# Ryukhaan/speech-to-video-mpp

Hardware: AMD Instinct MI355X
Metric: synthesized 256×256 frames/sec/GPU (LNet+ENet path); 1/2/4/8-GPU scaling (higher is better)
Workload: dtype f32; 1 GPU; ENet(+LNet) forward, B=16 synthetic 256x256 crops + [1,80,16] mel windows -> 384x384 (models/ENet.py:82-139); crop=256, global_batch=16, batch_per_gpu=16, parallelism=frame-shard x1 (no data-path collective), graph=True, lanes=1, world_size_seen=1

## Files before the change

### include/s2v.h

```cpp
#ifndef S2V_H_
#define S2V_H_

#include <stddef.h>
#include <stdint.h>

#ifdef __cplusplus
extern "C" {
#endif

typedef void *s2v_stream_t;

enum {
    S2V_OK = 0,
    S2V_E_INVALID = -1,
    S2V_E_LAUNCH = -2,
    S2V_E_WORKSPACE = -3
};

enum {
    S2V_ACT_NONE = 0,
    S2V_ACT_RELU = 1,
    S2V_ACT_LRELU = 2,
    S2V_ACT_SIGMOID = 3,
    S2V_ACT_TANH = 4,
// ... 85 lines not shown
                      float eps, float post, float *d, int d_ns, s2v_stream_t stream);

int s2v_modconv_demod_rows(const float *s, int batch, int s_ns, const int *rows, int nrows,
                           const float *wsq, float eps, float post, float *d, int d_ns,
                           s2v_stream_t stream);

int s2v_resize(const float *x, int n, int c, int ih, int iw, long long xsn, long long xsc, long long xsy,
               long long xsx, float *y, int oh, int ow, long long ysn, long long ysc, long long ysy,
               long long ysx, float scale_h, float scale_w, int mode, s2v_stream_t stream);

int s2v_torgb_up2(const float *x, int n, int h, int w, int c, int xcs, const float *wt, int kpad, const float *s,
                  int s_ns, const float *bias, const float *skip, int skcs, float *y, int ycs, s2v_stream_t stream);

typedef struct s2v_torgb_win {
    int fh, fw;
    int oy, ox;
    int sh, sw;
    int sy, sx;
    int nchw, cy, cx;
} s2v_torgb_win;
int s2v_torgb_up2_win(const float *x, int n, int h, int w, int c, int xcs, const float *wt, int kpad, const float *s,
                      int s_ns, const float *bias, const float *skip, int skcs, float *y, int ycs,
                      const s2v_torgb_win *win, s2v_stream_t stream);

int s2v_row_pack(const float *x, int n, int h, int w, int c, int xcs, int kw, int pw, float *y, int ycs,
                 s2v_stream_t stream);

int s2v_pad_reflect(const float *x, int n, int h, int w, int c, int xcs, int pt, int pb, int pl, int pr,
                    float *y, int ycs, s2v_stream_t stream);

int s2v_row_layernorm(const float *x, int rows, int dim, int xld, const float *weight, const float *bias,
                      float eps, float *y, int yld, s2v_stream_t stream);

int s2v_attention(const float *q, const float *k, const float *v, int batch, int heads, int tokens,
                  int dim_head, int ld_q, int ld_k, int ld_v, long long bs_q, long long bs_k, long long bs_v,
                  float scale, float *o, int ld_o, long long bs_o, s2v_stream_t stream);

int s2v_flow_warp(const float *flow, int n, int fh, int fw, int flow_cs, const float *src, int c, int h,
                  int w, long long ssn, long long ssc, long long ssy, long long ssx, float *y, int ycs,
                  s2v_stream_t stream);
int s2v_flow_warp_cat(const float *flow, int n, int fh, int fw, int flow_cs, const float *src, int c, int h,
                      int w, long long ssn, long long ssc, long long ssy, long long ssx, float *y, int ycs,
                      s2v_stream_t stream);

int s2v_melspectrogram(const float *wav, long long n_samples, const float *tables, int pad_reflect,
                       float *out, long long frames, s2v_stream_t stream);
// ... 186 lines not shown
```

### speech-to-video-mpp_amd/_lib.py

```python
from __future__ import annotations

import ctypes
import os
import threading

LIB_PATH = os.path.join(os.path.dirname(os.path.abspath(__file__)), "libs2v.so")

ACT_NONE, ACT_RELU, ACT_LRELU, ACT_SIGMOID, ACT_TANH, ACT_GELU_TANH = range(6)
IN_DIRECT, IN_NEAREST_UP2, IN_TRANSPOSED = range(3)
PAD_ZERO, PAD_REFLECT = range(2)
PREC_F32, PREC_BF16X3, PREC_F16X3, PREC_F16 = range(4)

_c_int, _c_float, _c_ll, _c_size, _vp = ctypes.c_int, ctypes.c_float, ctypes.c_longlong, ctypes.c_size_t, ctypes.c_void_p


class ConvParams(ctypes.Structure):
    _fields_ = [
        ("x", _vp), ("n", _c_int), ("h", _c_int), ("w", _c_int), ("cin", _c_int), ("xcs", _c_int),
        ("in_mode", _c_int), ("pad_mode", _c_int), ("pre_act", _c_int), ("pre_alpha", _c_float),
        ("in_scale", _vp), ("in_scale_ns", _c_int),
        ("kh", _c_int), ("kw", _c_int), ("sh", _c_int), ("sw", _c_int), ("ph", _c_int), ("pw", _c_int),
        ("dh", _c_int), ("dw", _c_int),
        ("wt", _vp), ("kpad", _c_int), ("npad", _c_int), ("cout", _c_int), ("b_kn", _c_int), ("ldb", _c_int),
        ("y", _vp), ("oh", _c_int), ("ow", _c_int), ("ycs", _c_int),
# ... 24 lines not shown
    "s2v_conv2d": (_c_int, [ctypes.POINTER(ConvParams), _vp]),
    "s2v_conv2d_ws_bytes": (_c_size, [ctypes.POINTER(ConvParams)]),
    "s2v_conv2d_plan": (_c_int, [ctypes.POINTER(ConvParams), ctypes.POINTER(_c_int)]),
    "s2v_conv2d_group": (_c_int, [ctypes.POINTER(ConvParams), _c_int, _vp]),
    "s2v_conv2d_group_ws_bytes": (_c_size, [ctypes.POINTER(ConvParams), _c_int]),
    "s2v_conv2d_group_plan": (_c_int, [ctypes.POINTER(ConvParams), _c_int, ctypes.POINTER(_c_int)]),
    "s2v_tune": (_c_int, [_c_int, _c_ll, ctypes.POINTER(_c_ll)]),
    "s2v_layernorm2d": (_c_int, [_vp, _c_int, _c_int, _c_int, _c_int, _c_int, _vp, _vp, _c_float, _c_int, _c_float,
                                 _c_int, _vp, _c_int, _vp, _c_int, _vp, _c_size, _vp]),
    "s2v_layernorm2d_ws_bytes": (_c_size, [_c_int, _c_int, _c_int, _c_int]),
    "s2v_instnorm_adain": (_c_int, [_vp, _c_int, _c_int, _c_int, _c_int, _c_int, _vp, _vp, _c_int, _c_float, _c_int,
                                    _c_float, _vp, _c_int, _vp, _c_int, _vp, _c_size, _vp]),
    "s2v_instnorm_adain_pad": (_c_int, [_vp, _c_int, _c_int, _c_int, _c_int, _c_int, _vp, _vp, _c_int, _c_float,
                                        _c_int, _c_float, _vp, _c_int, _vp, _c_int, _vp, _c_int, _vp, _c_size, _vp]),
    "s2v_instnorm_ws_bytes": (_c_size, [_c_int, _c_int, _c_int, _c_int]),
    "s2v_adain_params": (_c_int, [_vp, _c_int, _c_int, _c_int, _vp, _vp, _vp, _c_int, _vp, _c_int, _vp]),
    "s2v_modconv_demod": (_c_int, [_vp, _c_int, _c_int, _c_int, _vp, _c_int, _c_float, _c_float, _vp, _c_int, _vp]),
    "s2v_modconv_demod_rows": (_c_int, [_vp, _c_int, _c_int, _vp, _c_int, _vp, _c_float, _c_float, _vp, _c_int,
                                        _vp]),
    "s2v_torgb_up2": (_c_int, [_vp, _c_int, _c_int, _c_int, _c_int, _c_int, _vp, _c_int, _vp, _c_int, _vp, _vp,
                               _c_int, _vp, _c_int, _vp]),
    "s2v_torgb_up2_win": (_c_int, [_vp, _c_int, _c_int, _c_int, _c_int, _c_int, _vp, _c_int, _vp, _c_int, _vp, _vp,
                                   _c_int, _vp, _c_int, _vp, _vp]),
    "s2v_resize": (_c_int, [_vp, _c_int, _c_int, _c_int, _c_int, _c_ll, _c_ll, _c_ll, _c_ll, _vp, _c_int, _c_int,
                            _c_ll, _c_ll, _c_ll, _c_ll, _c_float, _c_float, _c_int, _vp]),
    "s2v_row_pack": (_c_int, [_vp, _c_int, _c_int, _c_int, _c_int, _c_int, _c_int, _c_int, _vp, _c_int, _vp]),
    "s2v_pad_reflect": (_c_int, [_vp, _c_int, _c_int, _c_int, _c_int, _c_int, _c_int, _c_int, _c_int, _c_int, _vp,
                                 _c_int, _vp]),
    "s2v_row_layernorm": (_c_int, [_vp, _c_int, _c_int, _c_int, _vp, _vp, _c_float, _vp, _c_int, _vp]),
    "s2v_attention": (_c_int, [_vp, _vp, _vp, _c_int, _c_int, _c_int, _c_int, _c_int, _c_int, _c_int, _c_ll, _c_ll,
                               _c_ll, _c_float, _vp, _c_int, _c_ll, _vp]),
    "s2v_flow_warp": (_c_int, [_vp, _c_int, _c_int, _c_int, _c_int, _vp, _c_int, _c_int, _c_int, _c_ll, _c_ll,
                               _c_ll, _c_ll, _vp, _c_int, _vp]),
    "s2v_flow_warp_cat": (_c_int, [_vp, _c_int, _c_int, _c_int, _c_int, _vp, _c_int, _c_int, _c_int, _c_ll, _c_ll,
                                   _c_ll, _c_ll, _vp, _c_int, _vp]),
    "s2v_melspectrogram": (_c_int, [_vp, _c_ll, _vp, _c_int, _vp, _c_ll, _vp]),
    "s2v_mel_chunks": (_c_int, [_vp, _c_ll, _vp, _c_int, _c_int, _vp, _vp]),
    "s2v_fused_bias_act": (_c_int, [_vp, _vp, _vp, _vp, _c_ll, _c_int, _c_ll, _c_int, _c_int, _c_float, _c_float,
                                    _vp]),
    "s2v_upfirdn2d": (_c_int, [_vp, _c_int, _c_int, _c_int, _c_int, _vp, _c_int, _c_int, _c_int, _c_int, _c_int,
                               _c_int, _c_int, _c_int, _c_int, _c_int, _vp, _c_int, _c_int, _vp]),
    "s2v_fused_bias_act_dt": (_c_int, [_c_int, _vp, _vp, _vp, _vp, _c_ll, _c_int, _c_ll, _c_int, _c_int,
                                       ctypes.c_double, ctypes.c_double, _vp]),
    "s2v_upfirdn2d_dt": (_c_int, [_c_int, _vp, _c_int, _c_int, _c_int, _c_int, _vp, _c_int, _c_int, _c_int, _c_int,
                                  _c_int, _c_int, _c_int, _c_int, _c_int, _c_int, _vp, _c_int, _c_int, _vp]),
    "s2v_fir2d": (_c_int, [_vp, _c_int, _c_int, _c_int, _c_int, _c_int, _vp, _c_int, _c_int, _c_int, _c_int, _c_int,
# ... 132 lines not shown
```

### speech-to-video-mpp_amd/csrc/torch_launch.cpp

```cpp
#include <ATen/ATen.h>
#include <ATen/hip/HIPContext.h>
#include <c10/core/DeviceGuard.h>
#include <torch/library.h>

#include <vector>

#include "../../include/s2v.h"

namespace {

using at::Tensor;
using OptT = c10::optional<Tensor>;

void *stream() { return (void *)at::hip::getCurrentHIPStream().stream(); }

void check(int rc, const char *what) { TORCH_CHECK(rc == 0, what, " failed (", rc, "): ", s2v_last_error()); }

bool has(const OptT &t) { return t && t->defined(); }

void same_dev(const Tensor &t, const at::Device &dev, const char *what) {
    TORCH_CHECK(t.is_cuda(), what, ": expected a HIP device tensor (the s2v ops have no CPU kernel)");
    TORCH_CHECK(t.device() == dev, what, ": on ", t.device(), ", the op's inputs are on ", dev);
}

// ... 674 lines not shown
    } else {
        for (int64_t v : window) TORCH_CHECK(v >= 0 && v < (1 << 30), "torgb window: bad value ", v);
        win.fh = (int)window[0]; win.fw = (int)window[1]; win.oy = (int)window[2]; win.ox = (int)window[3];
        win.sy = (int)window[4]; win.sx = (int)window[5];
    }
    float *yp = nullptr;
    int ycs = 0;
    if (crop.empty()) {
        const NV yv = nhwc(y, dev, "torgb y");
        TORCH_CHECK(yv.n == xv.n && yv.h == xv.h && yv.w == xv.w && yv.c == 4, "torgb: y [N, H, W, 4] view expected");
        yp = yv.p; ycs = yv.cs;
    } else {
        f32(y, dev, "torgb y");
        TORCH_CHECK(crop[0] >= 0 && crop[1] >= 0 && 2 * crop[0] < xv.h && 2 * crop[1] < xv.w, "torgb crop: bad (cy, cx)");
        win.nchw = 1; win.cy = (int)crop[0]; win.cx = (int)crop[1];
        TORCH_CHECK(y.dim() == 4 && y.is_contiguous() && y.size(0) == xv.n && y.size(1) == 3 &&
                        y.size(2) == xv.h - 2 * win.cy && y.size(3) == xv.w - 2 * win.cx,
                    "torgb: contiguous NCHW y [N, 3, H - 2 cy, W - 2 cx] expected, got ", y.sizes());
        yp = y.data_ptr<float>();
    }
    check(s2v_torgb_up2_win(xv.p, xv.n, xv.h, xv.w, xv.c, xv.cs, wt.data_ptr<float>(), (int)wt.size(1),
                            s.data_ptr<float>(), s_ns, bp, kv.p, kv.cs, yp, ycs, &win, stream()),
          "s2v_torgb_up2");
}

void flow_warp_(const Tensor &flow, const Tensor &src, const Tensor &y) {
    const c10::DeviceGuard guard(flow.device());
    const at::Device dev = flow.device();
    const NV fv = nhwc(flow, dev, "flow_warp flow"), yv = nhwc(y, dev, "flow_warp y");
    f32(src, dev, "flow_warp src");
    TORCH_CHECK(src.dim() == 4 && src.size(0) == fv.n && fv.c >= 2, "flow_warp: src [N, C, H, W], flow >= 2 channels");
    TORCH_CHECK(yv.n == fv.n && yv.h == src.size(2) && yv.w == src.size(3) && yv.c == src.size(1), "flow_warp: y shape");
    check(s2v_flow_warp(fv.p, fv.n, fv.h, fv.w, fv.cs, src.data_ptr<float>(), (int)src.size(1), (int)src.size(2),
                        (int)src.size(3), src.stride(0), src.stride(1), src.stride(2), src.stride(3), yv.p, yv.cs,
                        stream()),
          "s2v_flow_warp");
}

void flow_warp_cat_(const Tensor &flow, const Tensor &src, const Tensor &y) {
    const c10::DeviceGuard guard(flow.device());
    const at::Device dev = flow.device();
    const NV fv = nhwc(flow, dev, "flow_warp_cat flow"), yv = nhwc(y, dev, "flow_warp_cat y");
    f32(src, dev, "flow_warp_cat src");
    TORCH_CHECK(src.dim() == 4 && src.size(0) == fv.n && fv.c >= 2, "flow_warp_cat: src [N, C, H, W], flow >= 2 channels");
    TORCH_CHECK(yv.n == fv.n && yv.h == src.size(2) && yv.w == src.size(3) && yv.c == 2 * src.size(1),
                "flow_warp_cat: y [N, H, W, 2C]");
// ... 293 lines not shown
    m.def("group_abort_() -> ()", &group_abort_);
    m.def("group_end_(Tensor? ws, bool dry) -> int[]", &group_end_);
    m.def("gemm_kn_(Tensor a, Tensor b, Tensor(a!) out, int batch, int a_bs, int b_bs, int out_bs, Tensor? res, "
          "int res_bs, int act, float alpha, int prec, Tensor? ws, int force_tile, int force_splits, bool dry) -> int[]");
    m.def("split_weights_(Tensor w, Tensor(a!) out, int prec, float scale) -> ()");
    m.def("split_act_(Tensor x, Tensor(a!) out, int prec) -> ()");
    m.def("layernorm2d_(Tensor x, Tensor weight, Tensor bias, float eps, int act, float alpha, bool pool, "
          "Tensor? res, Tensor(a!) y, Tensor? ws) -> int");
    m.def("instnorm_(Tensor x, Tensor? gamma, Tensor? beta, float eps, int act, float alpha, Tensor? res, "
          "Tensor(a!) y, Tensor(b!)? pad_out, Tensor? ws) -> int");
    m.def("adain_params_(Tensor hid, int nhidden, Tensor w2t, Tensor bias, Tensor seg, Tensor(a!) out) -> ()");
    m.def("modconv_demod_(Tensor s, Tensor wsq, Tensor(a!) d, float eps, float post) -> ()");
    m.def("modconv_demod_rows_(Tensor s, Tensor rows, Tensor wsq, Tensor(a!) d, float eps, float post, "
          "int s_reach) -> ()");
    m.def("row_layernorm_(Tensor x, Tensor weight, Tensor bias, float eps, Tensor(a!) y) -> ()");
    m.def("attention_(Tensor q, Tensor k, Tensor v, Tensor(a!) out, int batch, int heads, int tokens, int dim_head, "
          "float scale) -> ()");
    m.def("resize_(Tensor x, int x_off, int[4] x_size, int[4] x_stride, Tensor(a!) y, int y_off, int[4] y_size, "
          "int[4] y_stride, float scale_h, float scale_w, int mode) -> ()");
    m.def("pad_reflect_(Tensor x, Tensor(a!) y, int[4] pads) -> ()");
    m.def("row_pack_(Tensor x, Tensor(a!) y, int kw, int pw) -> ()");
    m.def("torgb_up2_(Tensor x, Tensor wt, Tensor s, Tensor? bias, Tensor skip, Tensor(a!) y, int[] window, "
          "int[] crop) -> ()");
    m.def("flow_warp_(Tensor flow, Tensor src, Tensor(a!) y) -> ()");
    m.def("flow_warp_cat_(Tensor flow, Tensor src, Tensor(a!) y) -> ()");
    m.def("fill_value_(Tensor(a!) y, float value) -> ()");
    m.def("gaussian_noise_(Tensor(a!) y, int seed, int offset, Tensor? ctr, int shift) -> ()");
    m.def("counter_add_(Tensor(a!) ctr, int inc) -> ()");
    m.def("rfft2_(Tensor x, Tensor tables, Tensor(a!) spec) -> ()");
    m.def("irfft2_(Tensor spec, Tensor tables, Tensor? res, Tensor(a!) y) -> ()");
    m.def("ffc_spec_fwd_(Tensor x_g, Tensor w1, float wt_scale, float x_scale, Tensor? scale, Tensor? shift, "
          "Tensor tables, Tensor(a!) t1, Tensor(b!) spec, Tensor? flag, int prec) -> ()");
    m.def("ffc_spec_inv_(Tensor spec, Tensor wfu, float wt_scale, float x_scale, Tensor? scale, Tensor? shift, "
          "Tensor tables, Tensor t1, Tensor(a!) u, Tensor? flag, int prec) -> ()");
    m.def("ffc_norm_(Tensor(c!) y, Tensor u, Tensor w2, float wt_scale, float x_scale, Tensor? gamma, Tensor? beta, "
          "float eps, int act, float alpha, Tensor? res, Tensor(a!) out, Tensor(b!)? pad_out, Tensor? flag, int prec) -> ()");
    m.def("eltwise_(Tensor x, Tensor? mul, Tensor? add, Tensor? bias, float a, int act, float alpha, float post, "
          "Tensor(a!) y) -> ()");
    m.def("fir2d_(Tensor x, Tensor kernel, Tensor(a!) y, int up, int down, int pad_y0, int pad_x0, float gain, "
          "Tensor? bias, int act, float alpha, float post) -> ()");
    m.def("lipsync_inputs_(Tensor src, Tensor? fake, Tensor(a!) ref_u8, Tensor(b!) face6, Tensor(c!) gt) -> ()");
    m.def("to_u8_(Tensor x, Tensor(a!) y, float lo, float hi, float scale, float offset) -> ()");
    m.def("mel_chunks_(Tensor mel, Tensor starts, int step, Tensor(a!) out) -> ()");
    m.def("melspectrogram_(Tensor wav, Tensor tables, bool pad_reflect, Tensor(a!) out) -> ()");
}

TORCH_LIBRARY_IMPL(s2v, CUDA, m) {
    m.impl("conv2d_", &conv2d_);
    m.impl("modulated_conv2d_", &modulated_conv2d_);
    m.impl("modulate_weights_", &modulate_weights_);
    m.impl("gemm_kn_", &gemm_kn_);
    m.impl("split_weights_", &split_weights_);
    m.impl("amax_", &amax_);
    m.impl("split_act_", &split_act_);
    m.impl("layernorm2d_", &layernorm2d_);
    m.impl("instnorm_", &instnorm_);
    m.impl("adain_params_", &adain_params_);
    m.impl("modconv_demod_", &modconv_demod_);
    m.impl("modconv_demod_rows_", &modconv_demod_rows_);
    m.impl("row_layernorm_", &row_layernorm_);
    m.impl("attention_", &attention_);
    m.impl("resize_", &resize_);
    m.impl("pad_reflect_", &pad_reflect_);
    m.impl("row_pack_", &row_pack_);
    m.impl("torgb_up2_", &torgb_up2_);
    m.impl("flow_warp_", &flow_warp_);
    m.impl("flow_warp_cat_", &flow_warp_cat_);
    m.impl("fill_value_", &fill_value_);
    m.impl("gaussian_noise_", &gaussian_noise_);
    m.impl("counter_add_", &counter_add_);
    m.impl("rfft2_", &rfft2_);
    m.impl("irfft2_", &irfft2_);
    m.impl("ffc_spec_fwd_", &ffc_spec_fwd_);
    m.impl("ffc_spec_inv_", &ffc_spec_inv_);
    m.impl("ffc_norm_", &ffc_norm_);
    m.impl("eltwise_", &eltwise_);
    m.impl("fir2d_", &fir2d_);
    m.impl("lipsync_inputs_", &lipsync_inputs_);
    m.impl("to_u8_", &to_u8_);
    m.impl("mel_chunks_", &mel_chunks_);
    m.impl("melspectrogram_", &melspectrogram_);
}
```

### speech-to-video-mpp_amd/csrc/torgb.hip

```cpp
#include "common.hpp"

namespace s2v {

__host__ __device__ __forceinline__ void up2_index(int dst, int in, int &i0, int &i1, float &l0, float &l1) {
    float src = 0.5f * ((float)dst + 0.5f) - 0.5f;
    if (src < 0.f) src = 0.f;
    i0 = (int)src;
    i1 = i0 + ((i0 < in - 1) ? 1 : 0);
    l1 = src - (float)i0;
    l0 = 1.f - l1;
}


struct TorgbGeo {
    int fsh, fsw;
    int oy, ox;
    int sh, sw;
    int sy, sx;
    int nchw, cy, cx;
};

template <int TPP, int PPT>
__global__ __launch_bounds__(256) void torgb_up2_kernel(const float *__restrict__ x, int C, int H, int W, int xcs,
                                                        const float *__restrict__ wt, int kpad,
// ... 77 lines not shown
                yp[2 * plane] = r.z;
            }
        }
    }
}

template <int PPT>
static void launch_torgb(unsigned grid, size_t smem, const float *x, int c, int h, int w, int xcs, const float *wt,
                         int kpad, const float *s, int s_ns, const float *bias, const float *skip, int skcs, float *y,
                         int ycs, int chunks, const TorgbGeo &g, hipStream_t st) {
    torgb_up2_kernel<8, PPT><<<grid, 256, smem, st>>>(x, c, h, w, xcs, wt, kpad, s, s_ns, bias, skip, skcs, y, ycs,
                                                      chunks, g);
}

static void up2_tap_range(int o, int len, int in, int &lo, int &hi) {
    int i0, i1;
    float l0, l1;
    up2_index(o, in, i0, i1, l0, l1);
    lo = i0;
    up2_index(o + len - 1, in, i0, i1, l0, l1);
    hi = i1;
}

}

using namespace s2v;

extern "C" int s2v_torgb_up2_win(const float *x, int n, int h, int w, int c, int xcs, const float *wt, int kpad,
                                 const float *s, int s_ns, const float *bias, const float *skip, int skcs, float *y,
                                 int ycs, const s2v_torgb_win *win, s2v_stream_t stream) {
    S2V_REQUIRE(x && wt && s && skip && y && win && n > 0 && h > 1 && w > 1 && c > 0, "torgb_up2: bad args");
    const int fh = win->fh > 0 ? win->fh : h, fw = win->fw > 0 ? win->fw : w;
    S2V_REQUIRE(fh % 2 == 0 && fw % 2 == 0, "torgb_up2: output frame %dx%d must be twice the skip frame", fh, fw);
    S2V_REQUIRE(win->oy >= 0 && win->ox >= 0 && win->oy + h <= fh && win->ox + w <= fw,
                "torgb_up2: the %dx%d output window at (%d, %d) leaves the %dx%d frame", h, w, win->oy, win->ox, fh, fw);
    S2V_REQUIRE(win->sh > 0 && win->sw > 0 && win->sy >= 0 && win->sx >= 0 && win->sy + win->sh <= fh / 2 &&
                    win->sx + win->sw <= fw / 2,
                "torgb_up2: the %dx%d skip window at (%d, %d) leaves the %dx%d skip frame", win->sh, win->sw, win->sy,
                win->sx, fh / 2, fw / 2);
    int ylo, yhi, xlo, xhi;
    up2_tap_range(win->oy, h, fh / 2, ylo, yhi);
    up2_tap_range(win->ox, w, fw / 2, xlo, xhi);
    S2V_REQUIRE(ylo >= win->sy && yhi < win->sy + win->sh && xlo >= win->sx && xhi < win->sx + win->sw,
                "torgb_up2: the output window at (%d, %d) reads skip rows %d..%d, columns %d..%d: outside the %dx%d "
                "skip window at (%d, %d)", win->oy, win->ox, ylo, yhi, xlo, xhi, win->sh, win->sw, win->sy, win->sx);
    S2V_REQUIRE(c % 32 == 0 && xcs % 4 == 0 && xcs >= c && kpad >= c && s_ns >= c && skcs % 4 == 0 && skcs >= 4,
                "torgb_up2: C %% 32 == 0, 4-channel skip, float4 pitches required");
    S2V_REQUIRE(((uintptr_t)x % 16) == 0 && ((uintptr_t)skip % 16) == 0, "torgb_up2: 16-byte aligned x / skip");
    if (win->nchw)
// ... 35 lines not shown
```

### speech-to-video-mpp_amd/engine/enet.py

```python
from __future__ import annotations

import math
import os

import torch

from .. import ops
from ..ops import NHWC, ConvW
from .lnet import LNetEngine

LRELU = 0.2
OVERLAP = os.environ.get("S2V_ENET_OVERLAP", "1") == "1"
FUSED_TORGB = os.environ.get("S2V_ENET_FUSED_TORGB", "1") == "1"
POLY_UP = os.environ.get("S2V_ENET_POLY_UP", "1") == "1"
POLY_UP4 = os.environ.get("S2V_ENET_POLY_UP4", "0") == "1"
STYLE_GRID = os.environ.get("S2V_ENET_STYLE_GRID", "half")
ROWPACK0 = os.environ.get("S2V_ENET_ROWPACK0", "0") == "1"
FORK_AT = int(os.environ.get("S2V_ENET_FORK_AT", "0"))
PAUSE = tuple(int(v) for v in os.environ.get("S2V_ENET_PAUSE", "").split(":")) if os.environ.get("S2V_ENET_PAUSE") else None
PREMOD = os.environ.get("S2V_ENET_PREMOD", "1") == "1"
STACK_STRIPS = os.environ.get("S2V_ENET_STACK_STRIPS", "1") == "1"
RESUME_GRID = os.environ.get("S2V_ENET_RESUME_GRID", "")
CROP_TAIL = os.environ.get("S2V_ENET_CROP_TAIL", "1") == "1"
OUT_CROP = 8


def crop_tail_cone(size: int, crop: int):
    f1, f2 = 2 * size, 4 * size
    lo, hi = crop, f2 - 1 - crop
    if crop < 3 or lo > hi:
        return None
    need = {"rgb1": (lo, hi), "conv4": (lo, hi), "conv3": (lo - 1, hi + 1)}
    p0, p1 = (lo - 1) // 2, (hi + 1) // 2
    need["conv2"] = (p0 - 1, p1 + 1)
    need["conv1"] = (p0 - 2, p1 + 2)
    need["rgb0"] = ((2 * lo - 1) // 4, (2 * hi - 1) // 4 + 1)
    win = {"conv1": (1, f1 - 2), "conv2": (2, f1 - 4), "rgb0": (2, f1 - 4), "conv3": (6, f2 - 12),
           "conv4": (7, f2 - 14), "rgb1": (7, f2 - 14)}
    for k, (a, b) in need.items():
        o, n = win[k]
        if n <= 0 or a < o or b > o + n - 1:
            return None
    return {"need": need, "win": win, "crop": crop - 7, "out": f2 - 2 * crop}


def style_grid(device) -> int:
    if STYLE_GRID == "half":
        return ops.half_chip_blocks(device)
    return int(STYLE_GRID)

_FOLD = (((0.75, 0.25, 0.0), (0.25, 0.75, 0.75), (0.0, 0.0, 0.25)),
         ((0.25, 0.0, 0.0), (0.75, 0.75, 0.25), (0.0, 0.25, 0.75)))


def fold_up2_conv3(w: torch.Tensor) -> torch.Tensor:
    f = torch.tensor(_FOLD, dtype=torch.float64)
    wd = w.double()
    return torch.cat([torch.einsum("ap,bq,oipq->oiab", f[ry], f[rx], wd) for ry in (0, 1) for rx in (0, 1)]).float()


class StyleLayer:

    def __init__(self, sd, p, device, demodulate, upsample, is_rgb):
        m = p + "modulated_conv."
        w = sd[m + "weight"].float()[0]
        self.k = w.shape[-1]
        if w.shape[1] == 3:
            w = ops.pad_cin(w, 4)
        self.cin, self.cout = w.shape[1], w.shape[0]
        self.demodulate, self.upsample, self.is_rgb = demodulate, upsample, is_rgb
        bias = sd[p + "bias"].float().reshape(-1)
        self.conv = ConvW(w, bias, device, padding=self.k // 2)
        self.wsq = w.pow(2).sum((2, 3)).contiguous().to(device)
        self.mod_w = sd[m + "modulation.weight"].float()
        self.mod_b = sd[m + "modulation.bias"].float()
        if self.mod_w.shape[0] < self.cin:
            self.mod_w = torch.cat([self.mod_w, torch.zeros(self.cin - self.mod_w.shape[0], self.mod_w.shape[1])])
            self.mod_b = torch.cat([self.mod_b, torch.zeros(self.cin - self.mod_b.shape[0])])
        self.noise_w = None if is_rgb else float(sd[p + "weight"].float().reshape(-1)[0])
        self.device = device
        self.conv4 = self.wsq4 = None
        if upsample and self.k == 3 and (self.cin % 32 == 0 or (POLY_UP4 and self.cin == 4)):
            self.conv4 = ConvW(fold_up2_conv3(w), bias.repeat(4), device, padding=1)
            self.wsq4 = self.wsq.repeat(4, 1).contiguous()
        self.rp = None
        if ROWPACK0 and self.conv4 is None and not is_rgb and self.k == 3 and self.cin * self.k <= 32:
            self.conv.make_rowpack(device)
            self.rp = self.conv.rowpack.cin
            self.conv.rowpack.shift = self.conv.shift


class ENetEngine:
    def __init__(self, sd, device):
        dev = torch.device(device)
        self.device = dev
        self.lnet = LNetEngine(sd, dev, prefix="low_res.")
        self.first = ConvW(ops.pad_cin(sd["conv_body_first.weight"].float(), 4), sd["conv_body_first.bias"], dev)
        self.down = []
        for i in range(6):
            p = f"conv_body_down.{i}."
            sw = sd[p + "skip.weight"].float()
            skip2 = (sw / 4.0).expand(-1, -1, 2, 2).contiguous()
            self.down.append((ConvW(sd[p + "conv1.weight"], sd[p + "conv1.bias"], dev, padding=1),
                              ConvW(sd[p + "conv2.weight"], sd[p + "conv2.bias"], dev, padding=1),
                              ConvW(skip2, None, dev, stride=2)))
        self.final_conv = ConvW(sd["final_conv.weight"], sd["final_conv.bias"], dev, padding=1)
        wl = sd["final_linear.weight"].float()
        c4 = sd["final_conv.weight"].shape[0]
        wl = wl.reshape(wl.shape[0], c4, 4, 4).permute(0, 2, 3, 1).reshape(wl.shape[0], -1)
        self.final_linear = ConvW(wl, sd["final_linear.bias"], dev)
        self.layers = []
        for i in range(2):
            self.layers.append(StyleLayer(sd, f"style_convs.{2 * i}.", dev, True, True, False))
            self.layers.append(StyleLayer(sd, f"style_convs.{2 * i + 1}.", dev, True, False, False))
            self.layers.append(StyleLayer(sd, f"to_rgbs.{i}.", dev, False, False, True))
        offs, o, ws, bs = [], 0, [], []
        for l in self.layers:
            offs.append(o)
            mw, mb = l.mod_w, l.mod_b
            if l.rp is not None:
                z = l.rp - l.k * l.cin
                mw = torch.cat([mw] * l.k + [torch.zeros(z, mw.shape[1])])
                mb = torch.cat([mb] * l.k + [torch.zeros(z)])
            pad = (-mw.shape[0]) % 4
            ws += [mw, torch.zeros(pad, l.mod_w.shape[1])]
            bs += [mb, torch.zeros(pad)]
            o += mw.shape[0] + pad
        self.mod = ConvW(torch.cat(ws, 0), torch.cat(bs, 0), dev)
        self.mod_offs = offs
        self._demod = {}
        self.noise_seed = 0x5EED
        self.last_noises = [None] * 4

    def _side(self, ctx):
        side = ctx.streams(("enet", id(self)), 1)
        return None if side is None else side[0]

    def _demod_table(self, poly):
        if poly not in self._demod:
            ls = [(self.mod_offs[j], self.layers[j].wsq4 if poly and self.layers[j].conv4 is not None
                   else self.layers[j].wsq) for j in (0, 1, 3, 4)]
            t = ops.DemodRows(ls, self.device)
            t.width = [w.shape[0] for _, w in ls]
            self._demod[poly] = t
        return self._demod[poly]

    def _demods(self, ctx, s2):
        t = self._demod_table(POLY_UP)
        dall = ops.empty((s2.shape[0], t.nrows), self.device)
        ops.modconv_demod_rows(ctx, s2, t, dall, eps=1e-8, post=math.sqrt(2.0))
        return t, dall

    def _premodulate(self, ctx, s2, dtab, dall, b, strips=True) -> dict:
        wb = {}
        for st in range(2):
            for li in range(2):
                L, idx = self.layers[3 * st + li], 2 * st + li
                off = self.mod_offs[3 * st + li]
                r0, wd = dtab.r0[idx], dtab.width[idx]
                sv = s2[:, off: off + L.cin]
                if L.cin <= 4:
                    continue
                if POLY_UP and L.conv4 is not None:
                    d4 = dall[:, r0: r0 + wd]
                    wb[idx] = {"conv4": ops.modulate_weights(ctx, L.conv4, sv, d4, b)}
                    if strips:
                        wb[idx]["conv"] = ops.modulate_weights(ctx, L.conv, sv, d4[:, : L.cout], b)
                elif L.rp is None:
                    wb[idx] = {"conv": ops.modulate_weights(ctx, L.conv, sv, dall[:, r0: r0 + L.cout], b)}
        return wb

    def _poly_styleconv(self, ctx, L, cur: NHWC, s, d4, idx, noises, ctr, wb=None):
        dev, b = self.device, cur.n
        h2, w2 = 2 * cur.h, 2 * cur.w
        d = d4[:, : L.cout]
        noise = None
        if L.noise_w:
            if noises is not None and noises[idx] is not None:
                noise = noises[idx].reshape(b, h2, w2).contiguous()
            else:
                noise = torch.empty((b, h2, w2), device=dev)
                ops.gaussian_noise(ctx, noise, self.noise_seed, idx << 36, ctr=ctr, shift=40)
                self.last_noises[idx] = noise
        y = NHWC.empty(b, h2, w2, L.cout, dev)
        kw = dict(act=ops.ACT_LRELU, alpha=LRELU, pix_w=L.noise_w or 0.0)
        wb = wb or {}
        ops.modulated_conv2d(ctx, cur, L.conv4, y, s, d4, pix_add=noise, d2s=True, premod=wb.get("conv4"), **kw)
        c = cur.c
        if STACK_STRIPS:
            for axis, n_src, n_out in ((1, cur.h, h2), (2, cur.w, w2)):
                xs = NHWC(torch.cat([cur.t.narrow(axis, 0, 2), cur.t.narrow(axis, n_src - 2, 2)], axis))
                up = NHWC.empty(b, 2 * xs.h, 2 * xs.w, c, dev)
                ops.resize_nhwc(ctx, xs, up, scale_factor=2)
                ys = NHWC.empty(b, up.h, up.w, L.cout, dev)
                nz = None if noise is None else torch.cat([noise.narrow(axis, 0, 4), noise.narrow(axis, n_out - 4, 4)],
                                                          axis)
                ops.modulated_conv2d(ctx, up, L.conv, ys, s, d, pix_add=nz, premod=wb.get("conv"), **kw)
                y.t.narrow(axis, 0, 2).copy_(ys.t.narrow(axis, 0, 2))
                y.t.narrow(axis, n_out - 2, 2).copy_(ys.t.narrow(axis, 6, 2))
            return y
        strips = ((cur.t[:, 0:2], lambda t: t[:, 0:4], lambda t: t[:, 0:2], lambda t: t[:, 0:2]),
                  (cur.t[:, cur.h - 2:], lambda t: t[:, h2 - 4:], lambda t: t[:, 2:4], lambda t: t[:, h2 - 2:]),
                  (cur.t[:, :, 0:2], lambda t: t[:, :, 0:4], lambda t: t[:, :, 0:2], lambda t: t[:, :, 0:2]),
                  (cur.t[:, :, cur.w - 2:], lambda t: t[:, :, w2 - 4:], lambda t: t[:, :, 2:4],
                   lambda t: t[:, :, w2 - 2:]))
        for xs_t, nsel, ssel, ysel in strips:
            xs = NHWC(xs_t.contiguous())
            up = NHWC.empty(b, 2 * xs.h, 2 * xs.w, c, dev)
            ops.resize_nhwc(ctx, xs, up, scale_factor=2)
# ... 33 lines not shown
        def mod(j):
            sv = s2[:, self.mod_offs[j]: self.mod_offs[j] + L[j].cin]
            if L[j].is_rgb:
                return sv, None, {}
            idx = j - j // 3
            return sv, dtab.r0[idx], wbs.get(idx, {})

        x = NHWC.empty(b, f1, f1, cur.c, dev)
        ops.resize_nhwc(ctx, cur, x, scale_factor=2)
        for j, name in ((0, "conv1"), (1, "conv2")):
            o, n = win[name]
            s, r0, wb = mod(j)
            y = NHWC.empty(b, n, n, L[j].cout, dev)
            ops.modulated_conv2d(ctx, x, L[j].conv, y, s, dall[:, r0: r0 + L[j].cout], pix_w=L[j].noise_w or 0.0,
                                 pix_add=self._noise_window(ctx, L[j], j, b, f1, o, n, noises, ctr),
                                 premod=wb.get("conv"), **kw)
            x = y
        o, n = win["rgb0"]
        rgb0 = NHWC.empty(b, n, n, 4, dev)
        ops.torgb_up2(ctx, x, L[2].conv, mod(2)[0], cur, rgb0, frame=(f1, f1), origin=(o, o))
        o3, n3 = win["conv3"]
        s, r0, wb = mod(3)
        y = NHWC.empty(b, n3, n3, L[3].cout, dev)
        ops.modulated_conv2d(ctx, x, L[3].conv4, y, s, dall[:, r0: r0 + dtab.width[2]], d2s=True,
                             pix_w=L[3].noise_w or 0.0,
                             pix_add=self._noise_window(ctx, L[3], 2, b, f2, o3, n3, noises, ctr),
                             premod=wb.get("conv4"), **kw)
        o4, n4 = win["conv4"]
        s, r0, wb = mod(4)
        z = NHWC.empty(b, n4, n4, L[4].cout, dev)
        ops.modulated_conv2d(ctx, y, L[4].conv, z, s, dall[:, r0: r0 + L[4].cout], pix_w=L[4].noise_w or 0.0,
                             pix_add=self._noise_window(ctx, L[4], 3, b, f2, o4, n4, noises, ctr),
                             premod=wb.get("conv"), **kw)
        dst = out if out.is_contiguous() else torch.empty(out.shape, device=dev)
        ops.torgb_up2(ctx, z, L[5].conv, mod(5)[0], rgb0, dst, frame=(f2, f2), origin=(o4, o4), skip_origin=(o, o),
                      crop=(cone["crop"], cone["crop"]))
        if dst is not out:
            out.copy_(dst)

    def style_code(self, ctx, ref: torch.Tensor):
        st = self.style_begin(ctx, ref)
        self.style_down(ctx, st, len(self.down))
        return self.style_end(ctx, st)

    def style_begin(self, ctx, ref: torch.Tensor) -> dict:
        dev, b = self.device, ref.shape[0]
        x = NHWC.empty(b, 256, 256, 4, dev)
        ops.fill(ctx, x.t)
        ops.nchw_to_nhwc(ctx, ref, x.slice(0, 3))
        f = NHWC.empty(b, 256, 256, self.first.cout, dev)
# ... 140 lines not shown
```

### speech-to-video-mpp_amd/ops.py

```python
from __future__ import annotations

import contextlib
import ctypes
import math
import os
import threading
import weakref

import torch

from . import _lib, torch_ops
from ._lib import (ACT_GELU_TANH, ACT_LRELU, ACT_NONE, ACT_RELU, ACT_SIGMOID, ACT_TANH,
                   IN_DIRECT, IN_NEAREST_UP2, IN_TRANSPOSED, PAD_REFLECT, PAD_ZERO, PREC_BF16X3, PREC_F16, PREC_F16X3, PREC_F32,
                   check)

F32 = 4

_PRECISIONS = {"f16x3": PREC_F16X3, "bf16x3": PREC_BF16X3, "f32": PREC_F32, "f16": PREC_F16}
SPLIT_PRECISIONS = ("f16x3", "bf16x3")
PRECISION = os.environ.get("S2V_PRECISION", "f16x3")
if PRECISION not in _PRECISIONS:
    raise ValueError(f"S2V_PRECISION must be one of {sorted(_PRECISIONS)}, got {PRECISION!r}")


# ... 880 lines not shown
    off = x.coff + (crop[0] * x.w + crop[1]) * x.cs
    resize(ctx, x.t, off, (n, c, oh, ow), nhwc_strides(x), out, 0, (oh, ow), out.stride())
    return out


def torgb_up2(ctx: Ctx, x: NHWC, cw: "ConvW", s: torch.Tensor, skip: NHWC, y, *, frame=None, origin=(0, 0),
              skip_origin=(0, 0), crop=None):
    assert cw.kh == cw.kw == 1 and cw.cout == 3 and x.c == cw.cin, "torgb_up2: a 1x1 conv to 3 channels"
    assert skip.n == x.n and skip.c == 4
    if frame is None:
        assert origin == (0, 0) and skip_origin == (0, 0) and (2 * skip.h, 2 * skip.w) == (x.h, x.w)
        window = []
    else:
        window = [int(frame[0]), int(frame[1]), int(origin[0]), int(origin[1]), int(skip_origin[0]), int(skip_origin[1])]
    if crop is None:
        assert (y.n, y.h, y.w, y.c) == (x.n, x.h, x.w, 4)
        S2V.torgb_up2_(x.v, cw.wt, s, cw.shift, skip.v, y.v, window, [])
    else:
        assert tuple(y.shape) == (x.n, 3, x.h - 2 * crop[0], x.w - 2 * crop[1])
        S2V.torgb_up2_(x.v, cw.wt, s, cw.shift, skip.v, y, window, [int(crop[0]), int(crop[1])])
    return y


def row_pack(ctx: Ctx, x: NHWC, y: NHWC, kw: int, pw: int):
    S2V.row_pack_(x.v, y.v, kw, pw)
    return y


def pad_reflect(ctx: Ctx, x: NHWC, y: NHWC, pads):
    S2V.pad_reflect_(x.v, y.v, list(pads))
    return y


def row_layernorm(ctx: Ctx, x: torch.Tensor, weight, bias, y: torch.Tensor, eps=1e-5):
    S2V.row_layernorm_(x, weight, bias, eps, y)
    return y


def attention(ctx: Ctx, q: torch.Tensor, k: torch.Tensor, v: torch.Tensor, out: torch.Tensor, *, batch, heads,
              tokens, dim_head=64, scale=None):
    scale = dim_head ** -0.5 if scale is None else scale
    S2V.attention_(q, k, v, out, batch, heads, tokens, dim_head, scale)
    return out


def flow_warp(ctx: Ctx, flow: NHWC, src: torch.Tensor, y: NHWC):
# ... 145 lines not shown
```

Baseline: 701.9 frames/s.

## Replace upsample-then-conv3x3 with per-tap 1x1 products plus bilinear tap-sum kernel

For the upsampling style convs, the old path folded the 2x bilinear upsample into a 4-phase conv. The new path instead runs a 1x1 modulated conv at low resolution, producing nine tap-product blocks (9*Cout channels). A new HIP kernel then sums those blocks with fixed bilinear weights into the 2x output, fusing bias, noise and leaky ReLU. The aim is fewer MACs at high resolution, at the cost of a large 9*Cout intermediate written to and read back from memory, plus special handling at the frame edges.

```diff
diff --git a/include/s2v.h b/include/s2v.h
--- a/include/s2v.h
+++ b/include/s2v.h
@@ -131,6 +131,15 @@
 int s2v_torgb_up2_win(const float *x, int n, int h, int w, int c, int xcs, const float *wt, int kpad, const float *s,
                       int s_ns, const float *bias, const float *skip, int skcs, float *y, int ycs,
                       const s2v_torgb_win *win, s2v_stream_t stream);
+
+typedef struct s2v_tapsum_win {
+    int fh, fw;
+    int oy, ox;
+    int sy, sx;
+} s2v_tapsum_win;
+int s2v_tapsum_up2(const float *p, int n, int ph, int pw, int pcs, int cout, const float *noise, float pix_w,
+                   const float *bias, float gain, int act, float alpha, float *y, int oh, int ow, int ycs,
+                   const s2v_tapsum_win *win, s2v_stream_t stream);
 
 int s2v_row_pack(const float *x, int n, int h, int w, int c, int xcs, int kw, int pw, float *y, int ycs,
                  s2v_stream_t stream);
diff --git a/speech-to-video-mpp_amd/_lib.py b/speech-to-video-mpp_amd/_lib.py
--- a/speech-to-video-mpp_amd/_lib.py
+++ b/speech-to-video-mpp_amd/_lib.py
@@ -70,6 +70,8 @@
                                _c_int, _vp, _c_int, _vp]),
     "s2v_torgb_up2_win": (_c_int, [_vp, _c_int, _c_int, _c_int, _c_int, _c_int, _vp, _c_int, _vp, _c_int, _vp, _vp,
                                    _c_int, _vp, _c_int, _vp, _vp]),
+    "s2v_tapsum_up2": (_c_int, [_vp, _c_int, _c_int, _c_int, _c_int, _c_int, _vp, _c_float, _vp, _c_float, _c_int,
+                                _c_float, _vp, _c_int, _c_int, _c_int, _vp, _vp]),
     "s2v_resize": (_c_int, [_vp, _c_int, _c_int, _c_int, _c_int, _c_ll, _c_ll, _c_ll, _c_ll, _vp, _c_int, _c_int,
                             _c_ll, _c_ll, _c_ll, _c_ll, _c_float, _c_float, _c_int, _vp]),
     "s2v_row_pack": (_c_int, [_vp, _c_int, _c_int, _c_int, _c_int, _c_int, _c_int, _c_int, _vp, _c_int, _vp]),
diff --git a/speech-to-video-mpp_amd/csrc/torch_launch.cpp b/speech-to-video-mpp_amd/csrc/torch_launch.cpp
--- a/speech-to-video-mpp_amd/csrc/torch_launch.cpp
+++ b/speech-to-video-mpp_amd/csrc/torch_launch.cpp
@@ -720,6 +720,28 @@
     check(s2v_torgb_up2_win(xv.p, xv.n, xv.h, xv.w, xv.c, xv.cs, wt.data_ptr<float>(), (int)wt.size(1),
                             s.data_ptr<float>(), s_ns, bp, kv.p, kv.cs, yp, ycs, &win, stream()),
           "s2v_torgb_up2");
+}
+
+void tapsum_up2_(const Tensor &p, const OptT &noise, double pix_w, const OptT &bias, double gain, int64_t act,
+                 double alpha, const Tensor &y, at::IntArrayRef window) {
+    const c10::DeviceGuard guard(p.device());
+    const at::Device dev = p.device();
+    const NV pv = nhwc(p, dev, "tapsum p"), yv = nhwc(y, dev, "tapsum y");
+    TORCH_CHECK(yv.n == pv.n && pv.c == 9 * yv.c, "tapsum: p [N, PH, PW, 9 C] and y [N, OH, OW, C] views expected");
+    TORCH_CHECK(window.empty() || window.size() == 6, "tapsum window: (fh, fw, oy, ox, sy, sx) or empty");
+    s2v_tapsum_win win{};
+    if (window.empty()) {
+        TORCH_CHECK(yv.h == 2 * pv.h && yv.w == 2 * pv.w, "tapsum: y [N, 2 PH, 2 PW, C] expected");
+    } else {
+        for (int64_t v : window) TORCH_CHECK(v >= 0 && v < (1 << 29), "tapsum window: bad value ", v);
+        win.fh = (int)window[0]; win.fw = (int)window[1]; win.oy = (int)window[2]; win.ox = (int)window[3];
+        win.sy = (int)window[4]; win.sx = (int)window[5];
+    }
+    const float *np = vec(noise, dev, (int64_t)yv.n * yv.h * yv.w, "tapsum noise");
+    const float *bp = vec(bias, dev, yv.c, "tapsum bias");
+    check(s2v_tapsum_up2(pv.p, pv.n, pv.h, pv.w, pv.cs, yv.c, np, (float)pix_w, bp, (float)gain, (int)act, (float)alpha,
+                         yv.p, yv.h, yv.w, yv.cs, &win, stream()),
+          "s2v_tapsum_up2");
 }
 
 void flow_warp_(const Tensor &flow, const Tensor &src, const Tensor &y) {
@@ -1059,6 +1081,8 @@
     m.def("row_pack_(Tensor x, Tensor(a!) y, int kw, int pw) -> ()");
     m.def("torgb_up2_(Tensor x, Tensor wt, Tensor s, Tensor? bias, Tensor skip, Tensor(a!) y, int[] window, "
           "int[] crop) -> ()");
+    m.def("tapsum_up2_(Tensor p, Tensor? noise, float pix_w, Tensor? bias, float gain, int act, float alpha, "
+          "Tensor(a!) y, int[] window) -> ()");
     m.def("flow_warp_(Tensor flow, Tensor src, Tensor(a!) y) -> ()");
     m.def("flow_warp_cat_(Tensor flow, Tensor src, Tensor(a!) y) -> ()");
     m.def("fill_value_(Tensor(a!) y, float value) -> ()");
@@ -1101,6 +1125,7 @@
     m.impl("pad_reflect_", &pad_reflect_);
     m.impl("row_pack_", &row_pack_);
     m.impl("torgb_up2_", &torgb_up2_);
+    m.impl("tapsum_up2_", &tapsum_up2_);
     m.impl("flow_warp_", &flow_warp_);
     m.impl("flow_warp_cat_", &flow_warp_cat_);
     m.impl("fill_value_", &fill_value_);
diff --git a/speech-to-video-mpp_amd/csrc/torgb.hip b/speech-to-video-mpp_amd/csrc/torgb.hip
--- a/speech-to-video-mpp_amd/csrc/torgb.hip
+++ b/speech-to-video-mpp_amd/csrc/torgb.hip
@@ -123,9 +123,199 @@
     hi = i1;
 }
 
+struct TapsumGeo {
+    int fh, fw;
+    int ph, pw, sy, sx;
+    int oh, ow, oy, ox;
+    int k0, j0, ckh, ckw;
+};
+
+struct TapsumEpi {
+    const float *noise;
+    float pix_w;
+    const float *bias;
+    float gain;
+    int act;
+    float alpha;
+    float *y;
+    int ycs;
+};
+
+__device__ __forceinline__ constexpr float tapsum_w(int par, int ti) { return (par ^ ti) ? 0.25f : 0.75f; }
+
+template <int DY, int DX>
+__device__ __forceinline__ void tapsum_tap(const float *__restrict__ pt, const long long (&ro)[3], const long long (&co)[3],
+                                           float4 (&acc)[2][2]) {
+    constexpr int kLo[3] = {0, 0, 1}, kHi[3] = {1, 2, 2};
+    float4 v[3][3];
+#pragma unroll
+    for (int si = 0; si < 3; ++si)
+#pragma unroll
+        for (int sj = 0; sj < 3; ++sj)
+            if (si >= kLo[DY] && si <= kHi[DY] && sj >= kLo[DX] && sj <= kHi[DX])
+                v[si][sj] = *(const float4 *)(pt + ro[si] + co[sj]);
+#pragma unroll
+    for (int a = 0; a < 2; ++a)
+#pragma unroll
+        for (int c = 0; c < 2; ++c) {
+            const int bi = a + DY <= 1 ? 0 : 1, bj = c + DX <= 1 ? 0 : 1;
+#pragma unroll
+            for (int ti = 0; ti < 2; ++ti)
+#pragma unroll
+                for (int tj = 0; tj < 2; ++tj) {
+                    const float cf = tapsum_w((a + DY) & 1, ti) * tapsum_w((c + DX) & 1, tj);
+                    const float4 u = v[bi + ti][bj + tj];
+                    acc[a][c].x = fmaf(cf, u.x, acc[a][c].x);
+                    acc[a][c].y = fmaf(cf, u.y, acc[a][c].y);
+                    acc[a][c].z = fmaf(cf, u.z, acc[a][c].z);
+                    acc[a][c].w = fmaf(cf, u.w, acc[a][c].w);
+                }
+        }
+}
+
+__device__ __forceinline__ void tapsum_store(const TapsumEpi &e, const TapsumGeo &g, int b, int wr, int wc, int quad,
+                                             float4 acc) {
+    const long long pix = ((long long)b * g.oh + wr) * g.ow + wc;
+    float4 bv = make_float4(0.f, 0.f, 0.f, 0.f);
+    if (e.bias) bv = *(const float4 *)(e.bias + quad * 4);
+    const float nz = e.noise ? e.pix_w * e.noise[pix] : 0.f;
+    float4 r;
+    r.x = apply_act(e.gain * acc.x + bv.x + nz, e.act, e.alpha);
+    r.y = apply_act(e.gain * acc.y + bv.y + nz, e.act, e.alpha);
+    r.z = apply_act(e.gain * acc.z + bv.z + nz, e.act, e.alpha);
+    r.w = apply_act(e.gain * acc.w + bv.w + nz, e.act, e.alpha);
+    *(float4 *)(e.y + pix * e.ycs + quad * 4) = r;
+}
+
+__global__ __launch_bounds__(256) void tapsum_up2_kernel(const float *__restrict__ P, int pcs, int cout, int quads,
+                                                         long long items, TapsumEpi e, TapsumGeo g) {
+    const long long item = (long long)xcd_block(blockIdx.x, gridDim.x) * 256 + threadIdx.x;
+    if (item >= items) return;
+    const int quad = (int)(item % quads);
+    long long cell = item / quads;
+    const int cj = (int)(cell % g.ckw);
+    cell /= g.ckw;
+    const int ck = (int)(cell % g.ckh);
+    const int b = (int)(cell / g.ckh);
+    const int k = g.k0 + ck, j = g.j0 + cj;
+    const float *pb = P + (long long)b * g.ph * g.pw * pcs + quad * 4;
+    if (k >= 1 && k <= g.fh - 2 && j >= 1 && j <= g.fw - 2) {
+        long long ro[3], co[3];
+#pragma unroll
+        for (int s = 0; s < 3; ++s) {
+            ro[s] = (long long)min(max(k + s - 1 - g.sy, 0), g.ph - 1) * g.pw * pcs;
+            co[s] = (long long)min(max(j + s - 1 - g.sx, 0), g.pw - 1) * pcs;
+        }
+        float4 acc[2][2];
+#pragma unroll
+        for (int a = 0; a < 2; ++a)
+#pragma unroll
+            for (int c = 0; c < 2; ++c) acc[a][c] = make_float4(0.f, 0.f, 0.f, 0.f);
+#pragma unroll 1
+        for (int t = 0; t < 9; ++t) {
+            const float *pt = pb + t * cout;
+            switch (t) {
+                case 0: tapsum_tap<0, 0>(pt, ro, co, acc); break;
+                case 1: tapsum_tap<0, 1>(pt, ro, co, acc); break;
+                case 2: tapsum_tap<0, 2>(pt, ro, co, acc); break;
+                case 3: tapsum_tap<1, 0>(pt, ro, co, acc); break;
+                case 4: tapsum_tap<1, 1>(pt, ro, co, acc); break;
+                case 5: tapsum_tap<1, 2>(pt, ro, co, acc); break;
+                case 6: tapsum_tap<2, 0>(pt, ro, co, acc); break;
+                case 7: tapsum_tap<2, 1>(pt, ro, co, acc); break;
+                default: tapsum_tap<2, 2>(pt, ro, co, acc); break;
+            }
+        }
+#pragma unroll
+        for (int a = 0; a < 2; ++a)
+#pragma unroll
+            for (int c = 0; c < 2; ++c) {
+                const int wr = 2 * k + a - g.oy, wc = 2 * j + c - g.ox;
+                if ((unsigned)wr < (unsigned)g.oh && (unsigned)wc < (unsigned)g.ow) tapsum_store(e, g, b, wr, wc, quad, acc[a][c]);
+            }
+        return;
+    }
+#pragma unroll 1
+    for (int ac = 0; ac < 4; ++ac) {
+        const int r = 2 * k + (ac >> 1), c = 2 * j + (ac & 1);
+        const int wr = r - g.oy, wc = c - g.ox;
+        if ((unsigned)wr >= (unsigned)g.oh || (unsigned)wc >= (unsigned)g.ow) continue;
+        float4 acc = make_float4(0.f, 0.f, 0.f, 0.f);
+#pragma unroll 1
+        for (int t = 0; t < 9; ++t) {
+            const int qy = r + t / 3 - 1, qx = c + t % 3 - 1;
+            int i0, i1, j0, j1;
+            float ly[2], lx[2];
+            up2_index(qy, g.fh, i0, i1, ly[0], ly[1]);
+            up2_index(qx, g.fw, j0, j1, lx[0], lx[1]);
+            if (qy < 0 || qy >= 2 * g.fh) ly[0] = ly[1] = 0.f;
+            if (qx < 0 || qx >= 2 * g.fw) lx[0] = lx[1] = 0.f;
+            const long long rr[2] = {(long long)min(max(i0 - g.sy, 0), g.ph - 1) * g.pw * pcs,
+                                     (long long)min(max(i1 - g.sy, 0), g.ph - 1) * g.pw * pcs};
+            const long long cc[2] = {(long long)min(max(j0 - g.sx, 0), g.pw - 1) * pcs,
+                                     (long long)min(max(j1 - g.sx, 0), g.pw - 1) * pcs};
+            const float *pt = pb + t * cout;
+#pragma unroll
+            for (int ti = 0; ti < 2; ++ti)
+#pragma unroll
+                for (int tj = 0; tj < 2; ++tj) {
+                    const float cf = ly[ti] * lx[tj];
+                    const float4 u = *(const float4 *)(pt + rr[ti] + cc[tj]);
+                    acc.x = fmaf(cf, u.x, acc.x);
+                    acc.y = fmaf(cf, u.y, acc.y);
+                    acc.z = fmaf(cf, u.z, acc.z);
+                    acc.w = fmaf(cf, u.w, acc.w);
+                }
+        }
+        tapsum_store(e, g, b, wr, wc, quad, acc);
+    }
+}
+
 }
 
 using namespace s2v;
+
+extern "C" int s2v_tapsum_up2(const float *p, int n, int ph, int pw, int pcs, int cout, const float *noise, float pix_w,
+                              const float *bias, float gain, int act, float alpha, float *y, int oh, int ow, int ycs,
+                              const s2v_tapsum_win *win, s2v_stream_t stream) {
+    S2V_REQUIRE(p && y && win && n > 0 && ph > 0 && pw > 0 && oh > 0 && ow > 0 && cout > 0, "tapsum_up2: bad args");
+    S2V_REQUIRE(cout % 4 == 0, "tapsum_up2: Cout %d must be a multiple of 4 (16-byte channel accesses)", cout);
+    S2V_REQUIRE(act == S2V_ACT_NONE || act == S2V_ACT_LRELU || act == S2V_ACT_RELU, "tapsum_up2: unknown act %d", act);
+    const int fh = win->fh > 0 ? win->fh : ph, fw = win->fw > 0 ? win->fw : pw;
+    S2V_REQUIRE(fh < (1 << 29) && fw < (1 << 29), "tapsum_up2: frame too large");
+    S2V_REQUIRE(win->oy >= 0 && win->ox >= 0 && win->oy + (long long)oh <= 2LL * fh && win->ox + (long long)ow <= 2LL * fw,
+                "tapsum_up2: the %dx%d output window at (%d, %d) leaves the %dx%d frame", oh, ow, win->oy, win->ox,
+                2 * fh, 2 * fw);
+    S2V_REQUIRE(win->sy >= 0 && win->sx >= 0 && win->sy + (long long)ph <= fh && win->sx + (long long)pw <= fw,
+                "tapsum_up2: the %dx%d tap-product window at (%d, %d) leaves the %dx%d frame", ph, pw, win->sy, win->sx,
+                fh, fw);
+    int ylo, yhi, xlo, xhi;
+    {
+        const int qy0 = win->oy > 0 ? win->oy - 1 : 0, qy1 = win->oy + oh < 2 * fh ? win->oy + oh : 2 * fh - 1;
+        const int qx0 = win->ox > 0 ? win->ox - 1 : 0, qx1 = win->ox + ow < 2 * fw ? win->ox + ow : 2 * fw - 1;
+        up2_tap_range(qy0, qy1 - qy0 + 1, fh, ylo, yhi);
+        up2_tap_range(qx0, qx1 - qx0 + 1, fw, xlo, xhi);
+    }
+    S2V_REQUIRE(ylo >= win->sy && yhi < win->sy + ph && xlo >= win->sx && xhi < win->sx + pw,
+                "tapsum_up2: the output window at (%d, %d) reads tap-product rows %d..%d, columns %d..%d: outside the "
+                "%dx%d tap-product window at (%d, %d)", win->oy, win->ox, ylo, yhi, xlo, xhi, ph, pw, win->sy, win->sx);
+    S2V_REQUIRE(pcs % 4 == 0 && pcs >= 9LL * cout && ycs % 4 == 0 && ycs >= cout,
+                "tapsum_up2: pixel pitches must hold 9 Cout / Cout channels and be multiples of 4");
+    S2V_REQUIRE(((uintptr_t)p % 16) == 0 && ((uintptr_t)y % 16) == 0 && (!bias || ((uintptr_t)bias % 16) == 0),
+                "tapsum_up2: 16-byte aligned p / y / bias");
+    S2V_REQUIRE((long long)n * ph * pw * pcs < (1LL << 62) && (long long)n * oh * ow < (1LL << 40),
+                "tapsum_up2: problem too large");
+    const int k0 = win->oy >> 1, j0 = win->ox >> 1;
+    const int ckh = ((win->oy + oh - 1) >> 1) - k0 + 1, ckw = ((win->ox + ow - 1) >> 1) - j0 + 1;
+    const int quads = cout / 4;
+    const long long items = (long long)n * ckh * ckw * quads;
+    const long long blocks = (items + 255) / 256;
+    S2V_REQUIRE(blocks < (1LL << 31), "tapsum_up2: grid too large");
+    const TapsumGeo g{fh, fw, ph, pw, win->sy, win->sx, oh, ow, win->oy, win->ox, k0, j0, ckh, ckw};
+    const TapsumEpi e{noise, noise ? pix_w : 0.f, bias, gain, act, alpha, y, ycs};
+    tapsum_up2_kernel<<<(unsigned)blocks, 256, 0, (hipStream_t)stream>>>(p, pcs, cout, quads, items, e, g);
+    return check_launch("tapsum_up2");
+}
 
 extern "C" int s2v_torgb_up2_win(const float *x, int n, int h, int w, int c, int xcs, const float *wt, int kpad,
                                  const float *s, int s_ns, const float *bias, const float *skip, int skcs, float *y,
diff --git a/speech-to-video-mpp_amd/engine/enet.py b/speech-to-video-mpp_amd/engine/enet.py
--- a/speech-to-video-mpp_amd/engine/enet.py
+++ b/speech-to-video-mpp_amd/engine/enet.py
@@ -22,6 +22,8 @@
 STACK_STRIPS = os.environ.get("S2V_ENET_STACK_STRIPS", "1") == "1"
 RESUME_GRID = os.environ.get("S2V_ENET_RESUME_GRID", "")
 CROP_TAIL = os.environ.get("S2V_ENET_CROP_TAIL", "1") == "1"
+TAPSUM = os.environ.get("S2V_ENET_TAPSUM", "1") == "1"
+TAP_TILE = int(os.environ.get("S2V_ENET_TAP_TILE", "9"))
 OUT_CROP = 8
 
 
@@ -61,7 +63,7 @@
 
 class StyleLayer:
 
-    def __init__(self, sd, p, device, demodulate, upsample, is_rgb):
+    def __init__(self, sd, p, device, demodulate, upsample, is_rgb, tapsum=False):
         m = p + "modulated_conv."
         w = sd[m + "weight"].float()[0]
         self.k = w.shape[-1]
@@ -83,6 +85,10 @@
         if upsample and self.k == 3 and (self.cin % 32 == 0 or (POLY_UP4 and self.cin == 4)):
             self.conv4 = ConvW(fold_up2_conv3(w), bias.repeat(4), device, padding=1)
             self.wsq4 = self.wsq.repeat(4, 1).contiguous()
+        self.conv9 = self.wsq9 = None
+        if tapsum and self.conv4 is not None and self.cin % 32 == 0 and self.cout % 4 == 0:
+            self.conv9 = ConvW(w.permute(2, 3, 0, 1).reshape(9 * self.cout, self.cin, 1, 1), None, device)
+            self.wsq9 = self.wsq.repeat(9, 1).contiguous()
         self.rp = None
         if ROWPACK0 and self.conv4 is None and not is_rgb and self.k == 3 and self.cin * self.k <= 32:
             self.conv.make_rowpack(device)
@@ -111,7 +117,7 @@
         self.final_linear = ConvW(wl, sd["final_linear.bias"], dev)
         self.layers = []
         for i in range(2):
-            self.layers.append(StyleLayer(sd, f"style_convs.{2 * i}.", dev, True, True, False))
+            self.layers.append(StyleLayer(sd, f"style_convs.{2 * i}.", dev, True, True, False, tapsum=True))
             self.layers.append(StyleLayer(sd, f"style_convs.{2 * i + 1}.", dev, True, False, False))
             self.layers.append(StyleLayer(sd, f"to_rgbs.{i}.", dev, False, False, True))
         offs, o, ws, bs = [], 0, [], []
@@ -137,13 +143,17 @@
         return None if side is None else side[0]
 
     def _demod_table(self, poly):
-        if poly not in self._demod:
-            ls = [(self.mod_offs[j], self.layers[j].wsq4 if poly and self.layers[j].conv4 is not None
-                   else self.layers[j].wsq) for j in (0, 1, 3, 4)]
+        key = (poly, TAPSUM)
+        if key not in self._demod:
+            def rows(L):
+                if poly and TAPSUM and L.conv9 is not None:
+                    return L.wsq9
+                return L.wsq4 if poly and L.conv4 is not None else L.wsq
+            ls = [(self.mod_offs[j], rows(self.layers[j])) for j in (0, 1, 3, 4)]
             t = ops.DemodRows(ls, self.device)
             t.width = [w.shape[0] for _, w in ls]
-            self._demod[poly] = t
-        return self._demod[poly]
+            self._demod[key] = t
+        return self._demod[key]
 
     def _demods(self, ctx, s2):
         t = self._demod_table(POLY_UP)
@@ -161,7 +171,9 @@
                 sv = s2[:, off: off + L.cin]
                 if L.cin <= 4:
                     continue
-                if POLY_UP and L.conv4 is not None:
+                if POLY_UP and TAPSUM and L.conv9 is not None:
+                    wb[idx] = {"conv9": ops.modulate_weights(ctx, L.conv9, sv, dall[:, r0: r0 + wd], b)}
+                elif POLY_UP and L.conv4 is not None:
                     d4 = dall[:, r0: r0 + wd]
                     wb[idx] = {"conv4": ops.modulate_weights(ctx, L.conv4, sv, d4, b)}
                     if strips:
@@ -169,6 +181,15 @@
                 elif L.rp is None:
                     wb[idx] = {"conv": ops.modulate_weights(ctx, L.conv, sv, dall[:, r0: r0 + L.cout], b)}
         return wb
+
+    def _tapsum_styleconv(self, ctx, L, x: NHWC, s, d9, premod, noise, y: NHWC, frame=None, origin=(0, 0),
+                          src_origin=(0, 0)):
+        p = NHWC.empty(x.n, x.h, x.w, 9 * L.cout, self.device)
+        tile = TAP_TILE if ops.prec_code() != ops.PREC_F32 else 0
+        ops.modulated_conv2d(ctx, x, L.conv9, p, s, d9, premod=premod, force_tile=tile, force_splits=1)
+        ops.tapsum_up2(ctx, p, y, bias=L.conv.shift, pix_add=noise, pix_w=L.noise_w or 0.0, act=ops.ACT_LRELU,
+                       alpha=LRELU, frame=frame, origin=origin, src_origin=src_origin)
+        return y
 
     def _poly_styleconv(self, ctx, L, cur: NHWC, s, d4, idx, noises, ctr, wb=None):
         dev, b = self.device, cur.n
@@ -185,6 +206,8 @@
         y = NHWC.empty(b, h2, w2, L.cout, dev)
         kw = dict(act=ops.ACT_LRELU, alpha=LRELU, pix_w=L.noise_w or 0.0)
         wb = wb or {}
+        if TAPSUM and L.conv9 is not None:
+            return self._tapsum_styleconv(ctx, L, cur, s, d4, wb.get("conv9"), noise, y)
         ops.modulated_conv2d(ctx, cur, L.conv4, y, s, d4, pix_add=noise, d2s=True, premod=wb.get("conv4"), **kw)
         c = cur.c
         if STACK_STRIPS:
@@ -264,10 +287,14 @@
         o3, n3 = win["conv3"]
         s, r0, wb = mod(3)
         y = NHWC.empty(b, n3, n3, L[3].cout, dev)
-        ops.modulated_conv2d(ctx, x, L[3].conv4, y, s, dall[:, r0: r0 + dtab.width[2]], d2s=True,
-                             pix_w=L[3].noise_w or 0.0,
-                             pix_add=self._noise_window(ctx, L[3], 2, b, f2, o3, n3, noises, ctr),
-                             premod=wb.get("conv4"), **kw)
+        nz3 = self._noise_window(ctx, L[3], 2, b, f2, o3, n3, noises, ctr)
+        if TAPSUM and L[3].conv9 is not None:
+            o2 = win["conv2"][0]
+            self._tapsum_styleconv(ctx, L[3], x, s, dall[:, r0: r0 + dtab.width[2]], wb.get("conv9"), nz3, y,
+                                   frame=(f1, f1), origin=(o3, o3), src_origin=(o2, o2))
+        else:
+            ops.modulated_conv2d(ctx, x, L[3].conv4, y, s, dall[:, r0: r0 + dtab.width[2]], d2s=True,
+                                 pix_w=L[3].noise_w or 0.0, pix_add=nz3, premod=wb.get("conv4"), **kw)
         o4, n4 = win["conv4"]
         s, r0, wb = mod(4)
         z = NHWC.empty(b, n4, n4, L[4].cout, dev)
diff --git a/speech-to-video-mpp_amd/ops.py b/speech-to-video-mpp_amd/ops.py
--- a/speech-to-video-mpp_amd/ops.py
+++ b/speech-to-video-mpp_amd/ops.py
@@ -926,6 +926,27 @@
     return y
 
 
+def up2_tap_window(origin: int, size: int, frame: int):
+    q0, q1 = max(origin - 1, 0), min(origin + size, 2 * frame - 1)
+    lo = int(max(0.5 * (q0 + 0.5) - 0.5, 0.0))
+    hi = min(int(max(0.5 * (q1 + 0.5) - 0.5, 0.0)) + 1, frame - 1)
+    return lo, hi - lo + 1
+
+
+def tapsum_up2(ctx: Ctx, p: NHWC, y: NHWC, *, bias=None, pix_add=None, pix_w=0.0, gain=1.0, act=ACT_NONE, alpha=0.0,
+               frame=None, origin=(0, 0), src_origin=(0, 0)):
+    assert p.n == y.n and p.c == 9 * y.c, "tapsum_up2: p carries nine tap blocks of y's channels"
+    if frame is None:
+        assert origin == (0, 0) and src_origin == (0, 0) and (y.h, y.w) == (2 * p.h, 2 * p.w)
+        window = []
+    else:
+        window = [int(frame[0]), int(frame[1]), int(origin[0]), int(origin[1]), int(src_origin[0]), int(src_origin[1])]
+    if pix_add is not None:
+        assert tuple(pix_add.shape) == (y.n, y.h, y.w) and pix_add.is_contiguous()
+    S2V.tapsum_up2_(p.v, pix_add, float(pix_w), bias, float(gain), int(act), float(alpha), y.v, window)
+    return y
+
+
 def row_pack(ctx: Ctx, x: NHWC, y: NHWC, kw: int, pw: int):
     S2V.row_pack_(x.v, y.v, kw, pw)
     return y
```

After: 739.2 frames/s, median of 6. 1.05x the previous value.
